# BBCG/epialleleR

Hardware: AMD Instinct MI355X
Metric: Mreads/s generateCytosineReport (150 bp PE) (higher is better)
Workload: dtype u8

## Files before the change

epialleler_amd/csrc/cx_report.hip:

```cpp
#include "common.hpp"
#include "tile_common.hpp"
#include <stdio.h>
#include <stdlib.h>
#include <string.h>

namespace epi {

#ifndef EPI_CX_WG
#define EPI_CX_WG 512
#endif
#ifndef EPI_CX_T1
#define EPI_CX_T1 2048
#endif
constexpr int CX_WG = EPI_CX_WG;
constexpr int CX_T1 = EPI_CX_T1;
constexpr int CX_CH = 16;
constexpr int CX_FLUSH_ROWS = 255;
constexpr int CX_SLAB_COV = 12;

struct __attribute__((packed, aligned(1))) U4u { uint32_t x, y, z, w; };

#ifndef EPI_CX_ABLATE
#define EPI_CX_ABLATE 0
#endif

struct Cx2Args {
  RowCols c;
  int64_t xm_cap;
  const Tile *tiles;
  uint32_t fill4;
  ClassLut lut_r;
  ClassLut lut_rx, lut_sx;
  ClassLut lut_s;
  ThrParams thr;
  const uint32_t *thr_tab;
  uint32_t ctx_of_plane;
  int32_t *pass_out;
  uint32_t *pool_key, *pool_meth, *pool_unmeth;
  uint32_t pool_cap;
  uint32_t *cursor;
  uint32_t slot_rows, ovf_base;
  uint32_t *tile_nrow, *tile_base;
  int32_t *slab;
  int heavy_rows;
  int heavy_chunk;
  int heavy_first;
  uint32_t *heavy_count, *heavy_max;
  uint32_t *heavy_list;
  int32_t *heavy_slab;
  uint32_t *deep_count, *deep_list;
  const uint32_t *tile_list, *tile_list_count;
  uint32_t *dbg;
  int64_t nrows;
  const uint32_t *prev_off, *prev_nrow;
  uint32_t *mismatch;
  int32_t *out[6];
  int64_t out_cap;
};

template <int T, int NP, bool LEAN = false> struct Cx2Lds {
  static constexpr int Q = T / 4;
  static constexpr int N_NARROW = 2 * NP * Q;
  static constexpr int N_CORR = 2 * Q;
  static constexpr int N_WIDE = LEAN ? 16 : 2 * NP * T;
  static constexpr int N_COV = T;
  unsigned long long *narrow, *corr;
  uint32_t *wide, *cov;
  uint32_t tid;
};

__device__ __forceinline__ uint32_t cx2_lut(uint32_t w, const ClassLut &X, uint32_t low8) {
  const uint32_t sel = (w & 0x0F0F0F0Fu) | low8;
  return __builtin_amdgcn_perm(X.lo1, X.lo0, sel) ^ __builtin_amdgcn_perm(X.hi1, X.hi0, sel ^ 0x08080808u);
}

template <int G>
__device__ __forceinline__ uint32_t cx2_group_sum(uint32_t v) {
  v += (uint32_t)__builtin_amdgcn_update_dpp(0, (int)v, 0xB1, 0xF, 0xF, true);
  v += (uint32_t)__builtin_amdgcn_update_dpp(0, (int)v, 0x4E, 0xF, 0xF, true);
  if (G >= 8) v += (uint32_t)__builtin_amdgcn_update_dpp(0, (int)v, 0x141, 0xF, 0xF, true);
  if (G >= 16) v += (uint32_t)__builtin_amdgcn_update_dpp(0, (int)v, 0x140, 0xF, 0xF, true);
  if (G >= 32) v += __shfl_xor(v, 16, 64);
  if (G >= 64) v += __shfl_xor(v, 32, 64);
  return v;
}

__device__ __forceinline__ int cx2_threshold(uint32_t n_m, uint32_t n_u, uint32_t o_m, uint32_t o_u, const ThrParams &prm) {
  int res = 0;
  if (n_m != 0) {
    const unsigned n_all = n_m + n_u;
    if (!(n_all < prm.min_n_ctx)) {
      const double frac = (double)n_m / (double)n_all;
      if (!(frac < prm.min_ctx_meth_frac)) {
        res = 1;
        if (o_m > 0) {
          const unsigned o_all = o_m + o_u;
          const double ofrac = (double)o_m / (double)o_all;
          if (ofrac > prm.max_ooctx_meth_frac) res = 0;
        }
      }
    }
  }
  return res;
}

__device__ __forceinline__ int cx2_threshold_tab(uint32_t n_m, uint32_t n_u, uint32_t o_m, uint32_t o_u, const ThrParams &prm,
                                                 const uint32_t *__restrict__ tab) {
  const uint32_t n_all = n_m + n_u, o_all = o_m + o_u;
  const uint32_t least = tab[n_all] & 0xFFFFu, most = tab[o_all] >> 16;
  return n_m != 0u && !(n_all < prm.min_n_ctx) && n_m >= least && (o_m == 0u || o_m <= most);
}

__global__ __launch_bounds__(256) void k_thr_table(ThrParams prm, int32_t nmax, uint32_t *__restrict__ tab) {
  const int32_t n = (int32_t)(blockIdx.x * 256 + threadIdx.x);
  if (n > nmax) return;
  uint32_t least = 0xFFFFu, most = 0u;
  if (n >= 1) {
    int32_t lo = 1, hi = n + 1;
    while (lo < hi) {
      const int32_t m = (lo + hi) >> 1;
      const double frac = (double)(uint32_t)m / (double)(uint32_t)n;
      if (!(frac < prm.min_ctx_meth_frac)) hi = m; else lo = m + 1;
    }
    if (lo <= n) least = (uint32_t)lo;
    lo = 1; hi = n + 1;
    while (lo < hi) {
      const int32_t m = (lo + hi) >> 1;
      const double frac = (double)(uint32_t)m / (double)(uint32_t)n;
      if (frac > prm.max_ooctx_meth_frac) hi = m; else lo = m + 1;
    }
    most = (uint32_t)(lo - 1);
  }
  tab[n] = least | (most << 16);
}

struct Cx2Row {
  const uint8_t *base;
  int32_t rel, len;
  int32_t c0, clast;
  bool edge;
  int sidx, ps;
};

__device__ __forceinline__ void cx2_mask_from(int lo , uint32_t (&m)[4]) {
  const unsigned long long x = ~0ull << ((8 * lo) & 63);
  const bool low = lo < 8;
  const unsigned long long a = low ? x : 0ull, b = low ? ~0ull : x;
  m[0] = (uint32_t)a; m[1] = (uint32_t)(a >> 32); m[2] = (uint32_t)b; m[3] = (uint32_t)(b >> 32);
// ... 59 lines not shown
    if (x == 0x12345678u) atomicAdd(L.cov, 1u);
    return;
  }
  {
    uint32_t mf[4], ml[4];
    cx2_mask_from(cb == g.c0 ? (g.rel & 15) : 0, mf);
    cx2_mask_upto(((g.rel + g.len - 1) & 15) + 1, ml);
#pragma unroll
    for (int d = 0; d < 4; d++) { asm("" : "+v"(mf[d])); asm("" : "+v"(ml[d])); }
#pragma unroll
    for (int d = 0; d < 4; d++) w[0][d] = (w[0][d] & mf[d]) | (a.fill4 & ~mf[d]);
#pragma unroll
    for (int u = 0; u < NU; u++) {
      const bool last = cb + u * G == g.clast;
      if (__ballot(last) != 0ull) {
        const uint32_t keep = last ? 0u : 0xFFFFFFFFu;
#pragma unroll
        for (int d = 0; d < 4; d++) {
          const uint32_t m = ml[d] | keep;
          w[u][d] = (w[u][d] & m) | (a.fill4 & ~m);
        }
      }
    }
  }

  unsigned long long *nar = L.narrow + g.sidx * NP * Q + 4 * cb;
  unsigned long long *cor = L.corr + g.sidx * Q + 4 * cb;
  if constexpr (FUSED) {
    static_assert(NP == 1, "fused thresholding: one reported context, the thresholding context");
    uint32_t cls[4] = {0, 0, 0, 0}, fl = 0;
#pragma unroll
    for (int u = 0; u < NU; u++) {
#pragma unroll
      for (int d = 0; d < 4; d++) w[u][d] = (EPI_CX_ABLATE & 4) ? w[u][d] : cx2_lut(w[u][d], a.lut_sx, 0u);
      fl |= w[u][0] | w[u][1] | w[u][2] | w[u][3];
    }
    auto count = [&](auto masked) {
      constexpr bool MASKED = decltype(masked)::value;
      constexpr uint32_t EV = MASKED ? 0x55555555u : 0xFFFFFFFFu;
      uint32_t E = 0, O = 0;
#pragma unroll
      for (int u = 0; u < NU; u++) {
        const uint32_t t = (w[u][0] & EV) + (w[u][1] & EV) + (w[u][2] & EV);
        const uint32_t d3 = w[u][3] & EV;
        E += (t & 0x33333333u) + (d3 & 0x33333333u);
        O += ((t >> 2) & 0x33333333u) + ((d3 >> 2) & 0x33333333u);
        if (u % 3 == 2 || u == NU - 1) {
          cls[0] = __builtin_amdgcn_sad_u8(E & 0x0F0F0F0Fu, 0u, cls[0]);
          cls[2] = __builtin_amdgcn_sad_u8((E >> 4) & 0x0F0F0F0Fu, 0u, cls[2]);
          cls[1] = __builtin_amdgcn_sad_u8(O & 0x0F0F0F0Fu, 0u, cls[1]);
          cls[3] = __builtin_amdgcn_sad_u8((O >> 4) & 0x0F0F0F0Fu, 0u, cls[3]);
          E = 0; O = 0;
        }
      }
    };
    if constexpr (MODE != 2) {
      if (__builtin_expect(__ballot((fl & 0xAAAAAAAAu) != 0u) == 0ull, 1)) count(std::false_type{});
      else count(std::true_type{});
    }
    if constexpr (MODE == 1) {
#pragma unroll
      for (int k = 0; k < 4; k++) carry[k] += cls[k];
      return;
    }
    if constexpr (MODE == 0) {
      const uint32_t s01 = cx2_group_sum<G>(cls[0] | (cls[1] << 16)), s23 = cx2_group_sum<G>(cls[2] | (cls[3] << 16));
      const uint32_t n_all = s01 & 0xFFFFu, n_m = s01 >> 16;
      g.ps = a.thr_tab ? cx2_threshold_tab(n_m, n_all - n_m, s23 & 0xFFFFu, s23 >> 16, a.thr, a.thr_tab)
                       : cx2_threshold(n_m, n_all - n_m, s23 & 0xFFFFu, s23 >> 16, a.thr);
      if (a.pass_out && sub == 0 && (uint32_t)g.rel < (uint32_t)T) a.pass_out[rcur] = g.ps;
    }
    const uint32_t pm = g.ps ? 0x01010101u : 0u;
#pragma unroll
    for (int u = 0; u < NU; u++) {
      const bool inside = (uint32_t)(cb + u * G) < (uint32_t)C;
#pragma unroll
      for (int d = 0; d < 4; d++) {
        const uint32_t lo = w[u][d] & 0x01010101u, hi = (w[u][d] >> 2) & pm;
        if (lo != 0u && inside && !(EPI_CX_ABLATE & 2)) atomicAdd(nar + 4 * u * G + d, (unsigned long long)lo | ((unsigned long long)hi << 32));
      }
    }
    const uint32_t fsel = g.ps ? 0x0A0A0A0Au : 0xA0A0A0A0u;
    if (__builtin_expect((fl & fsel) != 0u, 0)) {
      const int sh = g.ps ? 1 : 5;
#pragma unroll
      for (int u = 0; u < NU; u++) {
        const bool inside = (uint32_t)(cb + u * G) < (uint32_t)C;
#pragma unroll
        for (int d = 0; d < 4; d++) {
          const uint32_t sk = (w[u][d] >> sh) & 0x01010101u, db = (w[u][d] >> (sh + 2)) & 0x01010101u;
          if ((sk | db) != 0u && inside) atomicAdd(cor + 4 * u * G + d, (unsigned long long)sk | ((unsigned long long)db << 32));
        }
      }
    }
  } else if constexpr (NP == 1 && G >= 16) {
    const bool passing = g.ps != 0;
    const uint32_t k77 = (a.ctx_of_plane & 255u) * 0x11111111u;
    const uint32_t rm = passing ? 0xDDDDDDDDu : 0x55555555u, rv = passing ? 0x99999999u : 0x11111111u;
    uint32_t clean = 0xFFFFFFFFu;
#pragma unroll
    for (int u = 0; u < NU; u++) {
      const bool inside = (uint32_t)(cb + u * G) < (uint32_t)C;
#pragma unroll
      for (int e = 0; e < 2; e++) {
        const uint32_t pk = (w[u][2 * e] & 0x0F0F0F0Fu) | ((w[u][2 * e + 1] << 4) & 0xF0F0F0F0u);
        const uint32_t z = ((pk & 0x77777777u) ^ k77) + 0x77777777u;
        const uint32_t np = ~z & 0x88888888u;
        const uint32_t t = (pk & rm) ^ rv;
        clean &= ((t & 0x77777777u) + 0x77777777u) | t;
        if (np != 0u && inside && !(EPI_CX_ABLATE & 2)) {
          const uint32_t up = passing ? np & ~pk : 0u;
          const uint32_t n0 = (np >> 3) & 0x01010101u, n1 = (np >> 7) & 0x01010101u;
          if (n0 != 0u) atomicAdd(nar + 4 * u * G + 2 * e, (unsigned long long)n0 | ((unsigned long long)((up >> 3) & 0x01010101u) << 32));
          if (n1 != 0u) atomicAdd(nar + 4 * u * G + 2 * e + 1, (unsigned long long)n1 | ((unsigned long long)((up >> 7) & 0x01010101u) << 32));
        }
      }
    }
    if (__builtin_expect((~clean & 0x88888888u) != 0u, 0)) {
      const uint32_t pick0 = passing ? 0u : 0x08080808u;
#pragma unroll
      for (int u = 0; u < NU; u++) {
        const bool inside = (uint32_t)(cb + u * G) < (uint32_t)C;
#pragma unroll
        for (int d = 0; d < 4; d++) {
          const uint32_t f = cx2_lut(w[u][d], a.lut_rx, pick0);
          const uint32_t sk = (f >> 6) & 0x01010101u, db = (f >> 7) & 0x01010101u;
          if ((sk | db) != 0u && inside) atomicAdd(cor + 4 * u * G + d, (unsigned long long)sk | ((unsigned long long)db << 32));
        }
      }
    }
  } else {
    const uint32_t pick0 = g.ps == 0 ? 0x08080808u : 0u;
    uint32_t fl = 0;
#pragma unroll
    for (int u = 0; u < NU; u++) {
      const bool inside = (uint32_t)(cb + u * G) < (uint32_t)C;
#pragma unroll
      for (int d = 0; d < 4; d++) {
        const uint32_t f = cx2_lut(w[u][d], a.lut_rx, pick0);
        w[u][d] = f;
        fl |= f;
#pragma unroll
        for (int p = 0; p < NP; p++) {
          const uint32_t lo = (f >> (2 * p)) & 0x01010101u, hi = (f >> (2 * p + 1)) & 0x01010101u;
          if (lo != 0u && inside && !(EPI_CX_ABLATE & 2))
            atomicAdd(nar + p * Q + 4 * u * G + d, (unsigned long long)lo | ((unsigned long long)hi << 32));
        }
      }
    }
    if (__builtin_expect((fl & 0xC0C0C0C0u) != 0u, 0)) {
#pragma unroll
      for (int u = 0; u < NU; u++) {
        const bool inside = (uint32_t)(cb + u * G) < (uint32_t)C;
#pragma unroll
        for (int d = 0; d < 4; d++) {
          const uint32_t sk = (w[u][d] >> 6) & 0x01010101u, db = (w[u][d] >> 7) & 0x01010101u;
          if ((sk | db) != 0u && inside) atomicAdd(cor + 4 * u * G + d, (unsigned long long)sk | ((unsigned long long)db << 32));
        }
      }
    }
  }
}

template <int T, int G, int NU, int NP, bool FUSED, int WG, class LT>
__device__ __forceinline__ void cx2_rows(const Cx2Args &a, const Tile &td, int row_lo, int row_hi, const LT &L) {
  constexpr int R = 64 / G, NW = WG / 64, C = T / CX_CH;
  const int lane = L.tid & 63, wave = L.tid >> 6;
  const int sub = lane & (G - 1), grp = lane / G;
  Tile tb = td;
  tb.row_hi = row_hi;
  int r = row_lo + wave * R + grp;
  RowVals v = cx_load_row(a.c, tb, r);
  for (int rbase = row_lo + wave * R; rbase < row_hi; rbase += NW * R) {
    const int rcur = r;
    if (!EPI_DEV_CHECK(a.dbg, !v.ok || (rcur >= 0 && rcur < a.nrows && v.len >= 0 && (v.sd == 1 || v.sd == 2 || v.len == 0)), 22, rcur, v.sd)) return;
    r += NW * R;
    RowVals nv;
    bool fetched = false;
    auto fetch_next = [&]() { if (!fetched) { nv = cx_load_row(a.c, tb, r); fetched = true; } };
    if (v.ok && v.len > 0 && (int32_t)((uint32_t)v.st - (uint32_t)td.pos0) + v.len > 0) {
      Cx2Row g;
      g.rel = (int32_t)((uint32_t)v.st - (uint32_t)td.pos0);
      g.len = v.len;
      g.c0 = g.rel >> 4;
      g.clast = (g.rel + v.len - 1) >> 4;
      g.base = a.c.xm + (v.o - g.rel);
      g.edge = v.o < CX_CH || v.o + v.len + CX_CH > a.xm_cap;
      g.sidx = v.sd - 1;
      g.ps = v.ps;
      if constexpr (FUSED) {
        if (__builtin_expect(__ballot(g.clast - g.c0 >= G * NU) == 0ull, 1)) {
          cx2_visit<T, G, NU, NP, true>(a, g, g.c0, g.clast, sub, rcur, L, fetch_next);
        } else {
          uint32_t cls[4] = {0, 0, 0, 0};
          for (int32_t cs = g.c0; __ballot(cs <= g.clast) != 0ull; cs += G * NU)
            cx2_visit<T, G, NU, NP, true, 1>(a, g, cs, g.clast, sub, rcur, L, fetch_next, cls);
          const uint32_t s01 = cx2_group_sum<G>(cls[0] | (cls[1] << 16)), s23 = cx2_group_sum<G>(cls[2] | (cls[3] << 16));
          const uint32_t n_all = s01 & 0xFFFFu, n_m = s01 >> 16;
          g.ps = a.thr_tab ? cx2_threshold_tab(n_m, n_all - n_m, s23 & 0xFFFFu, s23 >> 16, a.thr, a.thr_tab)
                           : cx2_threshold(n_m, n_all - n_m, s23 & 0xFFFFu, s23 >> 16, a.thr);
          if (a.pass_out && sub == 0 && (uint32_t)g.rel < (uint32_t)T) a.pass_out[rcur] = g.ps;
          const int32_t ca = g.c0 > 0 ? g.c0 : 0, cz = g.clast < C - 1 ? g.clast : C - 1;
          for (int32_t cs = ca; __ballot(cs <= cz) != 0ull; cs += G * NU)
            cx2_visit<T, G, NU, NP, true, 2>(a, g, cs, cz, sub, rcur, L, fetch_next);
        }
      } else {
        const int32_t ca = g.c0 > 0 ? g.c0 : 0, cz = g.clast < C - 1 ? g.clast : C - 1;
        if (__builtin_expect(__ballot(cz - ca >= G * NU) == 0ull, 1)) {
          cx2_visit<T, G, NU, NP, false>(a, g, ca, cz, sub, rcur, L, fetch_next);
        } else {
          for (int32_t cs = ca; __ballot(cs <= cz) != 0ull; cs += G * NU) cx2_visit<T, G, NU, NP, false>(a, g, cs, cz, sub, rcur, L, fetch_next);
        }
      }
      if (sub == 0) {
        const int32_t ca = g.rel > 0 ? g.rel : 0, cb = g.rel + v.len < T ? g.rel + v.len : T;
        const uint32_t unit = g.sidx ? 65536u : 1u;
        if (ca < cb && !(EPI_CX_ABLATE & 32)) { atomicAdd(L.cov + ca, unit); if (cb < T) atomicAdd(L.cov + cb, 0u - unit); }
      }
    } else if (FUSED && v.ok && sub == 0 && a.pass_out && (uint32_t)((uint32_t)v.st - (uint32_t)td.pos0) < (uint32_t)T) {
      a.pass_out[rcur] = 0;
    }
    fetch_next();
    v = nv;
  }
}

template <int T, int NP, bool LEAN, int WG>
__device__ __forceinline__ void cx2_flush(const Cx2Lds<T, NP, LEAN> &L) {
  constexpr int Q = Cx2Lds<T, NP, LEAN>::Q;
  if constexpr (!LEAN) {
    for (int i = L.tid; i < 2 * NP * Q; i += WG) {
      const unsigned long long v = L.narrow[i];
      if (v == 0ull) continue;
      L.narrow[i] = 0ull;
      const uint32_t lo = (uint32_t)v, hi = (uint32_t)(v >> 32);
      const int sp = i / Q, q = i - sp * Q;
      uint4 *wd = reinterpret_cast<uint4 *>(L.wide + sp * T + 4 * q);
      uint4 c = *wd;
      c.x += (lo & 255u) | ((hi & 255u) << 16);
      c.y += ((lo >> 8) & 255u) | (((hi >> 8) & 255u) << 16);
      c.z += ((lo >> 16) & 255u) | (((hi >> 16) & 255u) << 16);
      c.w += (lo >> 24) | ((hi >> 24) << 16);
      *wd = c;
    }
  }
  for (int i = L.tid; i < 2 * Q; i += WG) {
    const unsigned long long v = L.corr[i];
    if (v == 0ull) continue;
    L.corr[i] = 0ull;
    const uint32_t sk = (uint32_t)v, db = (uint32_t)(v >> 32);
    const int s = i / Q, q = i - s * Q;
    const int32_t unit = s ? 65536 : 1;
    int32_t prev = 0;
#pragma unroll
    for (int j = 0; j < 4; j++) {
      const int32_t d = (int32_t)((db >> (8 * j)) & 255u) - (int32_t)((sk >> (8 * j)) & 255u);
      if (d != prev) atomicAdd(L.cov + 4 * q + j, (uint32_t)((d - prev) * unit));
      prev = d;
    }
    if (prev != 0 && 4 * q + 4 < T) atomicAdd(L.cov + 4 * q + 4, (uint32_t)(-prev * unit));
  }
}

__device__ __forceinline__ uint32_t cx_pool_reserve(const Cx2Args &a, int tile, uint32_t n, bool *fits) {
  if (n <= a.slot_rows) { *fits = true; return (uint32_t)tile * a.slot_rows; }
  const uint32_t o = atomicAdd(a.cursor, n);
  *fits = (uint64_t)a.ovf_base + o + n <= a.pool_cap;
  return a.ovf_base + o;
}

__device__ __forceinline__ void cx_direct_none(const Cx2Args &a, int tile, uint32_t tid = threadIdx.x) {
  if (a.prev_off && tid == 0 && a.prev_nrow[tile] != 0u) atomicAdd(a.mismatch, 1u);
}

template <int T, int NP> struct CxSrcLds {
  const uint32_t *wide, *cov;
  __device__ __forceinline__ uint32_t any(int sd, int pos) const {
    uint32_t x = 0;
#pragma unroll
    for (int p = 0; p < NP; p++) x |= wide[(sd * NP + p) * T + pos];
    return x;
  }
  __device__ __forceinline__ void pair(int sd, int p, int pos, uint32_t *n, uint32_t *M) const {
    const uint32_t w = wide[(sd * NP + p) * T + pos];
    *n = w & 0xFFFFu; *M = w >> 16;
  }
  __device__ __forceinline__ uint32_t coverage(int sd, int pos) const { const uint32_t v = cov[pos]; return sd ? v >> 16 : v & 0xFFFFu; }
};
template <int QS> struct CxSrcU8 {
  const uint32_t *narrow;
  const uint32_t *cov;
  __device__ __forceinline__ uint32_t any(int sd, int pos) const {
    return (narrow[2 * (sd * QS + (pos >> 2))] >> (8 * (pos & 3))) & 255u;
  }
  __device__ __forceinline__ void pair(int sd, int, int pos, uint32_t *n, uint32_t *M) const {
    const uint2 c = *reinterpret_cast<const uint2 *>(narrow + 2 * (sd * QS + (pos >> 2)));
    *n = (c.x >> (8 * (pos & 3))) & 255u; *M = (c.y >> (8 * (pos & 3))) & 255u;
  }
  __device__ __forceinline__ uint32_t coverage(int sd, int pos) const { const uint32_t v = cov[pos]; return sd ? v >> 16 : v & 0xFFFFu; }
};
template <int T, int NP> struct CxSrcSlab {
  const int32_t *slab;
  const uint32_t *cov;
  __device__ __forceinline__ uint32_t any(int sd, int pos) const {
    uint32_t x = 0;
#pragma unroll
    for (int p = 0; p < NP; p++) x |= (uint32_t)slab[(2 * (sd * NP + p)) * T + pos];
    return x;
  }
  __device__ __forceinline__ void pair(int sd, int p, int pos, uint32_t *n, uint32_t *M) const {
    *n = (uint32_t)slab[(2 * (sd * NP + p)) * T + pos]; *M = (uint32_t)slab[(2 * (sd * NP + p) + 1) * T + pos];
  }
  __device__ __forceinline__ uint32_t coverage(int sd, int pos) const { return cov[sd * T + pos]; }
};

template <int T, int WG = CX_WG>
__device__ __forceinline__ void cx2_prefix(uint32_t *arr, uint32_t *s_scan, uint32_t tid = threadIdx.x) {
  constexpr int PPT = T / WG, NW = WG / 64;
  static_assert(PPT >= 1 && PPT <= 8, "prefix layout");
  const int lane = tid & 63, wave = tid >> 6;
  uint32_t x[PPT];
#pragma unroll
  for (int j = 0; j < PPT; j++) x[j] = arr[tid * PPT + j];
#pragma unroll
  for (int j = 1; j < PPT; j++) x[j] += x[j - 1];
  const uint32_t inc = wave_scan_u32(x[PPT - 1]);
  if (lane == 63) s_scan[wave] = inc;
  __syncthreads();
  uint32_t before = inc - x[PPT - 1];
#pragma unroll
  for (int w = 0; w < NW; w++) before += w < wave ? s_scan[w] : 0u;
#pragma unroll
  for (int j = 0; j < PPT; j++) arr[tid * PPT + j] = x[j] + before;
  __syncthreads();
}

template <int T, int NP, int WG = CX_WG, class SRC>
__device__ __forceinline__ void cx2_emit(const Cx2Args &a, int tile, const SRC &src, uint32_t *s_scan, uint16_t *s_list, uint32_t tid = threadIdx.x) {
  constexpr int NW = WG / 64, PW = T / NW, IT = PW / 32;
  static_assert(PW % 32 == 0 && IT >= 1 && IT <= 16, "emit phase layout");
  const int lane = tid & 63, wave = tid >> 6;
  const int l5 = lane & 31, sd = lane >> 5;
  const uint32_t below = (1u << l5) - 1u;
  uint16_t *list = s_list + wave * (2 * PW);
  uint32_t nc = 0;
#pragma unroll
  for (int i = 0; i < IT; i++) {
    const uint32_t any = src.any(sd, wave * PW + i * 32 + l5);
    const unsigned long long bal = __ballot(any != 0u);
    const uint32_t blo = (uint32_t)bal, bhi = (uint32_t)(bal >> 32);
    const uint32_t rank = (uint32_t)__popc(blo & below) + (uint32_t)__popc(bhi & below) + (sd ? (blo >> l5) & 1u : 0u);
    if (any != 0u) list[nc + rank] = (uint16_t)(i * 64 + lane);
    nc += (uint32_t)__popcll(bal);
  }
  uint32_t key[IT], me[IT], un[IT], off[IT];
  bool ok[IT];
  uint32_t carry = 0;
#pragma unroll
  for (int jj = 0; jj < IT; jj++) {
    ok[jj] = false; key[jj] = 0; me[jj] = 0; un[jj] = 0; off[jj] = 0;
    if ((uint32_t)(jj * 64) < nc) {
      const uint32_t j = (uint32_t)(jj * 64 + lane);
      bool good = false;
      if (j < nc) {
        const uint32_t id = list[j];
        const int pos = wave * PW + (int)(id >> 6) * 32 + (int)(id & 31u), st = (int)((id >> 5) & 1u);
        const uint32_t half = src.coverage(st, pos) >> 1;
        uint32_t ctx = 0, m = 0, u = 0;
#pragma unroll
        for (int p = 0; p < NP; p++) {
          uint32_t nn, M;
          src.pair(st, p, pos, &nn, &M);
          if (nn > half && ctx == 0) { ctx = (a.ctx_of_plane >> (8 * p)) & 255u; m = M; u = nn - M; }
        }
        good = ctx != 0;
        key[jj] = ((uint32_t)pos << 4) | ((uint32_t)st << 3) | ctx;
        me[jj] = m;
        un[jj] = u;
      }
      const unsigned long long be = __ballot(good);
      off[jj] = carry + __builtin_amdgcn_mbcnt_hi((uint32_t)(be >> 32), __builtin_amdgcn_mbcnt_lo((uint32_t)be, 0u));
      carry += (uint32_t)__popcll(be);
      ok[jj] = good;
    }
  }
  if (lane == 0) s_scan[wave] = carry;
  __syncthreads();
  if (a.prev_off) {
    if (tid == 0) {
      uint32_t acc = 0;
      for (int w = 0; w < NW; w++) { const uint32_t t = s_scan[w]; s_scan[w] = acc; acc += t; }
      const uint32_t base = a.prev_off[tile];
      const bool good = acc == a.prev_nrow[tile] && (int64_t)base + acc <= a.out_cap;
      if (!good) atomicAdd(a.mismatch, 1u);
      s_scan[NW + 1] = good ? base : 0xFFFFFFFFu;
    }
    __syncthreads();
    const uint32_t base = s_scan[NW + 1];
    if (base != 0xFFFFFFFFu) {
      const Tile td = a.tiles[tile];
      const uint32_t w0 = base + s_scan[wave];
#pragma unroll
      for (int jj = 0; jj < IT; jj++) {
        if (ok[jj]) {
          const uint32_t o = w0 + off[jj];
          a.out[0][o] = td.rname;
          a.out[1][o] = 1 + (int32_t)((key[jj] >> 3) & 1u);
          a.out[2][o] = (int32_t)(td.pos0 + (int64_t)(key[jj] >> 4));
          a.out[3][o] = (int32_t)(key[jj] & 7u);
          a.out[4][o] = (int32_t)me[jj];
          a.out[5][o] = (int32_t)un[jj];
        }
      }
    }
    return;
  }
  if (tid == 0) {
    uint32_t acc = 0;
    for (int w = 0; w < NW; w++) { const uint32_t t = s_scan[w]; s_scan[w] = acc; acc += t; }
    s_scan[NW] = acc;
    uint32_t base = 0;
    bool fits = true;
    if (acc) base = cx_pool_reserve(a, tile, acc, &fits);
    s_scan[NW + 1] = base;
    s_scan[NW] = fits ? acc : 0xFFFFFFFFu;
    a.tile_nrow[tile] = acc;
    a.tile_base[tile] = base;
  }
  __syncthreads();
  const uint32_t total = s_scan[NW], base = s_scan[NW + 1];
  if (total != 0xFFFFFFFFu) {
    const uint32_t w0 = base + s_scan[wave];
#pragma unroll
    for (int jj = 0; jj < IT; jj++) {
      if (ok[jj]) {
        const uint32_t w = w0 + off[jj];
        if (!EPI_DEV_CHECK(a.dbg, w < a.pool_cap, 23, w, a.pool_cap)) continue;
        a.pool_key[w] = key[jj];
        a.pool_meth[w] = me[jj];
        a.pool_unmeth[w] = un[jj];
      }
    }
  }
}

template <int T, int NP, bool LEAN, int WG>
__device__ __forceinline__ void cx2_dump_slab(const Cx2Lds<T, NP, LEAN> &L, int32_t *slab) {
  uint32_t *dst = reinterpret_cast<uint32_t *>(slab);
  if constexpr (LEAN) {
    constexpr int Q = Cx2Lds<T, NP, LEAN>::Q;
    for (int i = L.tid; i < 2 * NP * Q; i += WG) {
      const unsigned long long v = L.narrow[i];
      if (v == 0ull) continue;
      const uint32_t lo = (uint32_t)v, hi = (uint32_t)(v >> 32);
      const int sp = i / Q, q = i - sp * Q;
#pragma unroll
      for (int j = 0; j < 4; j++) {
        const uint32_t n = (lo >> (8 * j)) & 255u, M = (hi >> (8 * j)) & 255u;
        if (n) atomicAdd(dst + (2 * sp) * T + 4 * q + j, n);
        if (M) atomicAdd(dst + (2 * sp + 1) * T + 4 * q + j, M);
      }
    }
  } else {
    for (int i = L.tid; i < 2 * NP * T; i += WG) {
      const uint32_t v = L.wide[i];
      if (!v) continue;
      const int sp = i / T, p = i - sp * T;
      if (v & 0xFFFFu) atomicAdd(dst + (2 * sp) * T + p, v & 0xFFFFu);
      if (v >> 16) atomicAdd(dst + (2 * sp + 1) * T + p, v >> 16);
    }
  }
  for (int p = L.tid; p < T; p += WG) {
    const uint32_t v = L.cov[p];
    if (!v) continue;
    const int32_t lo = (int32_t)(int16_t)(v & 0xFFFFu);
    const int32_t hi = ((int32_t)v - lo) >> 16;
    if (lo) atomicAdd(dst + CX_SLAB_COV * T + p, (uint32_t)lo);
    if (hi) atomicAdd(dst + (CX_SLAB_COV + 1) * T + p, (uint32_t)hi);
  }
}

__device__ __forceinline__ int cx_tile_of_block(int b, int ntiles) {
  const int chunk = (ntiles + 7) >> 3;
  return (b & 7) * chunk + (b >> 3);
}

template <int T, int NP, bool LEAN = false> constexpr int cx2_lds_bytes() {
  using LdsT = Cx2Lds<T, NP, LEAN>;
  return (LdsT::N_NARROW + LdsT::N_CORR) * 8 + (LdsT::N_WIDE + LdsT::N_COV) * 4;
}
#ifndef EPI_CX_WPS
#define EPI_CX_WPS 8
#endif
template <int T, int NP, int NU = 3, bool LEAN = false, int WG = CX_WG> constexpr int cx2_waves_per_simd() {
  const int by_lds = (160 * 1024) / (cx2_lds_bytes<T, NP, LEAN>() + 64), by_thr = 2048 / WG;
  int wgs = by_lds < by_thr ? by_lds : by_thr;
  if (NU >= 4 && wgs * WG > 1536) wgs = 1536 / WG;
  if (wgs * WG / 256 > EPI_CX_WPS) wgs = EPI_CX_WPS * 256 / WG;
  return (wgs < 1 ? 1 : wgs) * WG / 256;
}

#define CX2_SHARED(T, NP, LEAN)                                                                                  \
  using LdsT = Cx2Lds<T, NP, LEAN>;                                                                              \
  __shared__ __attribute__((aligned(16))) unsigned long long s_u8[LdsT::N_NARROW + LdsT::N_CORR];                \
  __shared__ __attribute__((aligned(16))) uint32_t s_wide[LdsT::N_WIDE];                                         \
  __shared__ __attribute__((aligned(16))) uint32_t s_cov[LdsT::N_COV];                                           \
  static_assert((LdsT::N_NARROW + LdsT::N_CORR) * 8 >= 4 * T + 64 && LdsT::N_CORR * 8 >= 4 * T, "the candidate lists and the scan scratch reuse dead arrays"); \
  uint32_t *s_scan = LEAN ? s_wide : reinterpret_cast<uint32_t *>(s_u8) + T;                                      \
  uint16_t *s_list = reinterpret_cast<uint16_t *>(LEAN ? s_u8 + LdsT::N_NARROW : s_u8);                          \
  (void)s_scan; (void)s_list;                                                                                     \
  LdsT L;                                                                                                         \
  L.narrow = s_u8; L.corr = s_u8 + LdsT::N_NARROW; L.wide = s_wide; L.cov = s_cov; L.tid = threadIdx.x;

template <int T, int NP, bool LEAN, int WG>
__device__ __forceinline__ void cx2_clear(const Cx2Lds<T, NP, LEAN> &L) {
  using LdsT = Cx2Lds<T, NP, LEAN>;
  uint4 *z = reinterpret_cast<uint4 *>(L.narrow);
  for (int i = L.tid; i < (LdsT::N_NARROW + LdsT::N_CORR) / 2; i += WG) z[i] = make_uint4(0, 0, 0, 0);
  if constexpr (!LEAN) {
    uint4 *y = reinterpret_cast<uint4 *>(L.wide);
    for (int i = L.tid; i < LdsT::N_WIDE / 4; i += WG) y[i] = make_uint4(0, 0, 0, 0);
  }
  uint4 *x = reinterpret_cast<uint4 *>(L.cov);
  for (int i = L.tid; i < LdsT::N_COV / 4; i += WG) x[i] = make_uint4(0, 0, 0, 0);
}

template <int T, int G, int NU, int NP, bool FUSED, bool LEAN, int WG>
__device__ __forceinline__ void cx2_accumulate(const Cx2Args &a, const Tile &td, int row_lo, int row_hi, const Cx2Lds<T, NP, LEAN> &L) {
  if constexpr (LEAN) {
    cx2_rows<T, G, NU, NP, FUSED, WG>(a, td, row_lo, row_hi, L);
  } else {
    for (int b0 = row_lo; b0 < row_hi; b0 += CX_FLUSH_ROWS) {
      if (b0 > row_lo) { __syncthreads(); cx2_flush<T, NP, LEAN, WG>(L); __syncthreads(); }
      cx2_rows<T, G, NU, NP, FUSED, WG>(a, td, b0, b0 + CX_FLUSH_ROWS < row_hi ? b0 + CX_FLUSH_ROWS : row_hi, L);
    }
  }
  __syncthreads();
  cx2_flush<T, NP, LEAN, WG>(L);
  __syncthreads();
}

#ifndef EPI_CX_LEAN_WG
#define EPI_CX_LEAN_WG 256
#endif
template <bool LEAN> constexpr int cx2_wg() { return LEAN ? EPI_CX_LEAN_WG : CX_WG; }

template <int T, int G, int NU, int NP, bool FUSED, bool LEAN, class LdsT>
__device__ __forceinline__ void cx2_tile(const Cx2Args &a, int tile, const Tile &td, const LdsT &L, uint32_t *s_scan, uint16_t *s_list, int *s_flag) {
  constexpr int WG = cx2_wg<LEAN>();
  cx2_clear<T, NP, LEAN, WG>(L);
  if (td.row_hi - td.row_lo > a.heavy_rows) {
    if (L.tid == 0) {
      const uint32_t h = atomicAdd(a.heavy_count, 1u);
      a.heavy_list[h] = (uint32_t)tile;
      atomicMax(a.heavy_max, (uint32_t)(td.row_hi - td.row_lo));
      a.tile_nrow[tile] = 0;
      a.tile_base[tile] = 0;
    }
    cx_direct_none(a, tile, L.tid);
    return;
  }
  if constexpr (LEAN) {
    if (a.deep_list && td.row_hi - td.row_lo > CX_FLUSH_ROWS) {
      if (L.tid == 0) *s_flag = 0;
      __syncthreads();
      bool deep = false;
      for (int x = td.row_lo + (int)L.tid; x + CX_FLUSH_ROWS < td.row_hi; x += WG)
        deep |= (int64_t)a.c.start[x + CX_FLUSH_ROWS] < (int64_t)a.c.start[x] + a.c.len[x];
      if (deep) *s_flag = 1;
      __syncthreads();
      if (*s_flag) {
        if (L.tid == 0) { a.deep_list[atomicAdd(a.deep_count, 1u)] = (uint32_t)tile; a.tile_nrow[tile] = 0; a.tile_base[tile] = 0; }
        cx_direct_none(a, tile, L.tid);
        return;
      }
    }
  }
  __syncthreads();
  cx2_accumulate<T, G, NU, NP, FUSED, LEAN, WG>(a, td, td.row_lo, td.row_hi, L);
  if (td.slot >= 0) {
    cx2_dump_slab<T, NP, LEAN, WG>(L, a.slab + (int64_t)td.slot * (kCxPlanes * T));
    if (L.tid == 0) { a.tile_nrow[tile] = 0; a.tile_base[tile] = 0; }
    cx_direct_none(a, tile, L.tid);
    return;
  }
  if (EPI_CX_ABLATE & 16) { if (L.tid == 0) { a.tile_nrow[tile] = 0; a.tile_base[tile] = 0; } cx_direct_none(a, tile, L.tid); return; }
  cx2_prefix<T, WG>(L.cov, s_scan, L.tid);
  if constexpr (LEAN) {
    static_assert(NP == 1, "the u8 counters serve single-context reports");
    CxSrcU8<LdsT::Q> src;
    src.narrow = reinterpret_cast<const uint32_t *>(L.narrow); src.cov = L.cov;
    cx2_emit<T, NP, WG>(a, tile, src, s_scan, s_list, L.tid);
  } else {
    CxSrcLds<T, NP> src;
    src.wide = L.wide; src.cov = L.cov;
    cx2_emit<T, NP, WG>(a, tile, src, s_scan, s_list, L.tid);
  }
}

template <int T, int G, int NU, int NP, bool FUSED, bool LEAN>
__global__ __launch_bounds__(cx2_wg<LEAN>(), (cx2_waves_per_simd<T, NP, NU, LEAN, cx2_wg<LEAN>()>())) void k_cx_tiles(Cx2Args a, int ntiles) {
  CX2_SHARED(T, NP, LEAN)
  __shared__ int s_flag;
  if constexpr (!LEAN) {
    if (a.tile_list) {
      const uint32_t n = *a.tile_list_count;
      for (uint32_t i = blockIdx.x; i < n; i += gridDim.x) {
        const int tile = (int)a.tile_list[i];
        const Tile td = a.tiles[tile];
        cx2_tile<T, G, NU, NP, FUSED, LEAN>(a, tile, td, L, s_scan, s_list, &s_flag);
        __syncthreads();
      }
      return;
    }
  }
  const int tile = cx_tile_of_block(blockIdx.x, ntiles);
  if (tile >= ntiles) return;
  const Tile td = a.tiles[tile];
  cx2_tile<T, G, NU, NP, FUSED, LEAN>(a, tile, td, L, s_scan, s_list, &s_flag);
}

template <int T, int G, int NU, int NP, bool FUSED>
__global__ __launch_bounds__(CX_WG, (cx2_waves_per_simd<T, NP, NU>())) void k_cx_heavy(Cx2Args a) {
  CX2_SHARED(T, NP, false)
  const uint32_t hi_idx = (uint32_t)a.heavy_first + blockIdx.y;
  if (hi_idx >= *a.heavy_count) return;
  const int tile = (int)a.heavy_list[hi_idx];
  const Tile td = a.tiles[tile];
  for (int lo = td.row_lo + (int)blockIdx.x * a.heavy_chunk; lo < td.row_hi; lo += (int)gridDim.x * a.heavy_chunk) {
    const int hi = td.row_hi - lo > a.heavy_chunk ? lo + a.heavy_chunk : td.row_hi;
    cx2_clear<T, NP, false, CX_WG>(L);
    __syncthreads();
    cx2_accumulate<T, G, NU, NP, FUSED, false, CX_WG>(a, td, lo, hi, L);
    cx2_dump_slab<T, NP, false, CX_WG>(L, td.slot >= 0 ? a.slab + (int64_t)td.slot * (kCxPlanes * T)
                                          : a.heavy_slab + (int64_t)blockIdx.y * (kCxPlanes * T));
    __syncthreads();
  }
}

template <int T, int NP>
__device__ __forceinline__ void cx2_emit_from_slab(const Cx2Args &a, int tile, const int32_t *slab) {
  __shared__ __attribute__((aligned(16))) uint32_t s_cov[2 * T];
  __shared__ uint32_t s_scan[CX_WG / 64 + 2];
  __shared__ uint16_t s_list[2 * T];
  for (int i = threadIdx.x; i < 2 * T; i += CX_WG) s_cov[i] = (uint32_t)slab[CX_SLAB_COV * T + i];
  __syncthreads();
  cx2_prefix<T>(s_cov, s_scan);
  cx2_prefix<T>(s_cov + T, s_scan);
  CxSrcSlab<T, NP> src;
  src.slab = slab; src.cov = s_cov;
  cx2_emit<T, NP>(a, tile, src, s_scan, s_list);
}

template <int T, int NP>
__global__ __launch_bounds__(CX_WG) void k_cx_emit_heavy(Cx2Args a) {
  const uint32_t hi_idx = (uint32_t)a.heavy_first + blockIdx.x;
  if (hi_idx >= *a.heavy_count) return;
  const int tile = (int)a.heavy_list[hi_idx];
  if (a.tiles[tile].slot >= 0) return;
  cx2_emit_from_slab<T, NP>(a, tile, a.heavy_slab + (int64_t)blockIdx.x * (kCxPlanes * T));
}

template <int T, int NP>
__global__ __launch_bounds__(CX_WG) void k_cx_emit_slab(Cx2Args a, const int32_t *__restrict__ owned,
                                                         const int32_t *__restrict__ slot_tile) {
  if (!owned[blockIdx.x]) return;
  const int tile = slot_tile[blockIdx.x];
  if (tile < 0) return;
  cx2_emit_from_slab<T, NP>(a, tile, a.slab + (int64_t)a.tiles[tile].slot * (kCxPlanes * T));
}

#ifndef EPI_CXP_T
#define EPI_CXP_T 1024
#endif
constexpr int CXP_T = EPI_CXP_T;

template <int G, int U0, int U1>
__device__ __forceinline__ void cxp_add_range(const uint32_t (&w)[CX_NU], const RowSlice &cur) {
  if constexpr (U0 < U1) {
    if (U0 * G <= cur.tl) cx_add_dword<CXP_T, 4 * G * U0, U0 == 0>(w[U0], cur.tl == U0 * G, cur);
    cxp_add_range<G, U0 + 1, U1>(w, cur);
  }
}

template <int G>
__device__ __forceinline__ void cxp_accumulate(const RowCols &c, const Tile &td, uint32_t *cnt) {
  constexpr int R = 64 / G, NW = CX_WG / 64;
  const int lane = threadIdx.x & 63, wave = threadIdx.x >> 6;
  const int sub = lane & (G - 1), grp = lane / G;
  int r = td.row_lo + wave * R + grp;
  RowSlice cur = cx_row_slice<CXP_T, G>(c, td, r, sub, cnt);
  for (int rbase = td.row_lo + wave * R; rbase < td.row_hi; rbase += NW * R) {
    uint32_t w[CX_NU];
#pragma unroll
    for (int u = 0; u < CX_NU; u++) w[u] = u * G <= cur.tl ? cur.src[u * G] : 0u;
    r += NW * R;
    const RowSlice nxt = cx_row_slice<CXP_T, G>(c, td, r, sub, cnt);
    cxp_add_range<G, 0, CX_NU>(w, cur);
    for (int k = sub + CX_NU * G; k < cur.nd; k += G) {
      RowSlice t = cur;
#pragma unroll
      for (int j = 0; j < 4; j++) t.dst[j] = cur.dst[j] + 4 * (k - sub);
      cx_add_dword<CXP_T, 0, false>(cur.src[k - sub], k == cur.nd - 1, t);
    }
    cur = nxt;
  }
}

__device__ __forceinline__ void cxp_convert(uint32_t *cnt) {
  constexpr int T = CXP_T;
  for (int i = threadIdx.x; i < 2 * T; i += CX_WG) {
    uint32_t *c0 = cnt + (i / T) * 4 * T + (i % T);
    const uint32_t d0 = c0[0], dh = c0[T], dx = c0[2 * T], dz = c0[3 * T];
    const uint32_t nh = (dh & 0xFFFFu) + (dh >> 16), nx = (dx & 0xFFFFu) + (dx >> 16), nz = (dz & 0xFFFFu) + (dz >> 16);
    c0[0] = (d0 & 0xFFFFu) + (d0 >> 16) + nh + nx + nz;
    c0[T] = nh | (dh << 16);
    c0[2 * T] = nx | (dx << 16);
    c0[3 * T] = nz | (dz << 16);
  }
}

struct CxSrcPk {
  const uint32_t *cnt;
  int pl[3];
  __device__ __forceinline__ uint32_t any(int sd, int pos) const {
    uint32_t x = 0;
#pragma unroll
    for (int p = 0; p < 3; p++) if (pl[p]) x |= cnt[(sd * 4 + pl[p]) * CXP_T + pos];
    return x;
  }
  __device__ __forceinline__ void pair(int sd, int p, int pos, uint32_t *n, uint32_t *M) const {
    const uint32_t w = pl[p] ? cnt[(sd * 4 + pl[p]) * CXP_T + pos] : 0u;
    *n = w & 0xFFFFu; *M = w >> 16;
  }
  __device__ __forceinline__ uint32_t coverage(int sd, int pos) const { return cnt[sd * 4 * CXP_T + pos]; }
};

__device__ __forceinline__ CxSrcPk cxp_source(const Cx2Args &a, const uint32_t *cnt) {
  CxSrcPk s;
  s.cnt = cnt;
#pragma unroll
  for (int p = 0; p < 3; p++) { const uint32_t k = (a.ctx_of_plane >> (8 * p)) & 255u; s.pl[p] = k == 2u ? 1 : k == 6u ? 2 : k == 7u ? 3 : 0; }
  return s;
}

__device__ __forceinline__ void cxp_dump_slab(const Cx2Args &a, const uint32_t *cnt, int np, int32_t *slab) {
  constexpr int T = CXP_T;
  uint32_t *dst = reinterpret_cast<uint32_t *>(slab);
  const CxSrcPk src = cxp_source(a, cnt);
  for (int i = threadIdx.x; i < 2 * T; i += CX_WG) {
    const int sd = i / T, pos = i % T;
#pragma unroll
    for (int p = 0; p < 3; p++) {
      if (p >= np) break;
      uint32_t n, M;
      src.pair(sd, p, pos, &n, &M);
      if (n) atomicAdd(dst + (2 * (sd * np + p)) * T + pos, n);
      if (M) atomicAdd(dst + (2 * (sd * np + p) + 1) * T + pos, M);
    }
    const uint32_t d = src.coverage(sd, pos) - (pos ? src.coverage(sd, pos - 1) : 0u);
    if (d) atomicAdd(dst + (CX_SLAB_COV + sd) * T + pos, d);
  }
}

#define CXP_SHARED                                                                                      \
  __shared__ __attribute__((aligned(16))) uint32_t cnt_raw[8 * CXP_T + 2 * kCxGuard];                  \
  __shared__ uint32_t s_scan[CX_WG / 64 + 2];                                                         \
  __shared__ uint16_t s_list[2 * CXP_T];                                                               \
  uint32_t *cnt = cnt_raw + kCxGuard;

template <int G>
__global__ __launch_bounds__(CX_WG, 8) void k_cxp_tiles(Cx2Args a, int ntiles, int np) {
  CXP_SHARED
  const int tile = cx_tile_of_block(blockIdx.x, ntiles);
  if (tile >= ntiles) return;
  const Tile td = a.tiles[tile];
  uint4 *z = reinterpret_cast<uint4 *>(cnt_raw);
  for (int i = threadIdx.x; i < (8 * CXP_T + 2 * kCxGuard) / 4; i += CX_WG) z[i] = make_uint4(0, 0, 0, 0);
  if (td.row_hi - td.row_lo > a.heavy_rows) {
    if (threadIdx.x == 0) {
      const uint32_t h = atomicAdd(a.heavy_count, 1u);
      a.heavy_list[h] = (uint32_t)tile;
      atomicMax(a.heavy_max, (uint32_t)(td.row_hi - td.row_lo));
      a.tile_nrow[tile] = 0;
      a.tile_base[tile] = 0;
    }
    cx_direct_none(a, tile);
    return;
  }
  __syncthreads();
  cxp_accumulate<G>(a.c, td, cnt);
  __syncthreads();
  cxp_convert(cnt);
  __syncthreads();
  if (td.slot >= 0) {
    cxp_dump_slab(a, cnt, np, a.slab + (int64_t)td.slot * (kCxPlanes * CXP_T));
    if (threadIdx.x == 0) { a.tile_nrow[tile] = 0; a.tile_base[tile] = 0; }
    cx_direct_none(a, tile);
    return;
  }
  if (EPI_CX_ABLATE & 16) {
    if (threadIdx.x == 0) { a.tile_nrow[tile] = 0; a.tile_base[tile] = 0; }
    cx_direct_none(a, tile);
    return;
  }
  cx2_emit<CXP_T, 3>(a, tile, cxp_source(a, cnt), s_scan, s_list);
}

template <int G>
__global__ __launch_bounds__(CX_WG, 8) void k_cxp_heavy(Cx2Args a, int np) {
  CXP_SHARED
  (void)s_scan; (void)s_list;
  const uint32_t hi_idx = (uint32_t)a.heavy_first + blockIdx.y;
  if (hi_idx >= *a.heavy_count) return;
  const int tile = (int)a.heavy_list[hi_idx];
  const Tile whole = a.tiles[tile];
  for (int lo = whole.row_lo + (int)blockIdx.x * a.heavy_chunk; lo < whole.row_hi; lo += (int)gridDim.x * a.heavy_chunk) {
    Tile td = whole;
    td.row_lo = lo;
    if (td.row_hi - lo > a.heavy_chunk) td.row_hi = lo + a.heavy_chunk;
    uint4 *z = reinterpret_cast<uint4 *>(cnt_raw);
    for (int i = threadIdx.x; i < (8 * CXP_T + 2 * kCxGuard) / 4; i += CX_WG) z[i] = make_uint4(0, 0, 0, 0);
    __syncthreads();
    cxp_accumulate<G>(a.c, td, cnt);
    __syncthreads();
    cxp_convert(cnt);
    __syncthreads();
    cxp_dump_slab(a, cnt, np, td.slot >= 0 ? a.slab + (int64_t)td.slot * (kCxPlanes * CXP_T)
                                            : a.heavy_slab + (int64_t)blockIdx.y * (kCxPlanes * CXP_T));
    __syncthreads();
  }
}

struct __attribute__((packed, aligned(4))) CxU4u { uint32_t x, y, z, w; };

__global__ __launch_bounds__(256) void k_cx_gather(const Tile *__restrict__ tiles, const uint32_t *__restrict__ tile_out,
                                                    const uint32_t *__restrict__ tile_nrow, const uint32_t *__restrict__ tile_base,
                                                    int32_t ntiles, const uint32_t *__restrict__ pool_key,
                                                    const uint32_t *__restrict__ pool_meth, const uint32_t *__restrict__ pool_unmeth,
                                                    int32_t *__restrict__ o_rname, int32_t *__restrict__ o_strand,
                                                    int32_t *__restrict__ o_pos, int32_t *__restrict__ o_ctx,
                                                    int32_t *__restrict__ o_meth, int32_t *__restrict__ o_unmeth) {
  const int tile = blockIdx.x * 4 + (threadIdx.x >> 6);
  if (tile >= ntiles) return;
  const uint32_t n = tile_nrow[tile];
  if (n == 0) return;
  const int lane = threadIdx.x & 63;
  const Tile td = tiles[tile];
  const uint32_t src0 = tile_base[tile], dst0 = tile_out[tile];
  const uint32_t n4 = n & ~3u;
  for (uint32_t i = 4u * lane; i < n4; i += 256) {
    const CxU4u key = *reinterpret_cast<const CxU4u *>(pool_key + src0 + i);
    const CxU4u me = *reinterpret_cast<const CxU4u *>(pool_meth + src0 + i);
    const CxU4u un = *reinterpret_cast<const CxU4u *>(pool_unmeth + src0 + i);
    const uint32_t o = dst0 + i;
    const uint32_t rn = (uint32_t)td.rname;
    const uint32_t p0 = (uint32_t)td.pos0;
    *reinterpret_cast<CxU4u *>(o_rname + o) = CxU4u{rn, rn, rn, rn};
    *reinterpret_cast<CxU4u *>(o_strand + o) = CxU4u{1u + ((key.x >> 3) & 1u), 1u + ((key.y >> 3) & 1u), 1u + ((key.z >> 3) & 1u), 1u + ((key.w >> 3) & 1u)};
    *reinterpret_cast<CxU4u *>(o_pos + o) = CxU4u{p0 + (key.x >> 4), p0 + (key.y >> 4), p0 + (key.z >> 4), p0 + (key.w >> 4)};
    *reinterpret_cast<CxU4u *>(o_ctx + o) = CxU4u{key.x & 7u, key.y & 7u, key.z & 7u, key.w & 7u};
    *reinterpret_cast<CxU4u *>(o_meth + o) = me;
    *reinterpret_cast<CxU4u *>(o_unmeth + o) = un;
  }
  for (uint32_t i = n4 + lane; i < n; i += 64) {
    const uint32_t key = pool_key[src0 + i];
    const uint32_t o = dst0 + i;
    o_rname[o] = td.rname;
    o_strand[o] = 1 + (int32_t)((key >> 3) & 1u);
    o_pos[o] = (int32_t)(td.pos0 + (int64_t)(key >> 4));
    o_ctx[o] = (int32_t)(key & 7u);
    o_meth[o] = (int32_t)pool_meth[src0 + i];
    o_unmeth[o] = (int32_t)pool_unmeth[src0 + i];
  }
}


static int cx_tile_for(int np) { return np <= 1 ? CX_T1 : CXP_T; }

static int pick_cx_shape(const RowStats &st, int T, bool fused, bool lean) {
#ifdef EPI_CX_FORCE_SHAPE
  if (fused) return EPI_CX_FORCE_SHAPE;
#endif
  const int max_chunks = (int)(((int64_t)st.max_len + 2 * (CX_CH - 1)) / CX_CH);
  const int tile_chunks = T / CX_CH;
  double total = 0;
  for (int k = 0; k < kLenBinCount; k++) total += st.len_hist[k];
  int best = 64 * 8 + 3;
  double best_cost = -1;
// ... 662 lines not shown
```

Measured before the change: 12820.

## Skip lean correction flush when unused; hoist kept-offset loads and drop emit barrier

Adds an LDS flag in the lean layout that records whether any correction atomics fired, and skips the flush pass and its barrier when none did. The per-tile previous offset and row count are now loaded once at kernel entry and passed into emit. The serial thread-0 scan in emit, with its extra __syncthreads, is replaced by each wave reading all wave totals itself. The goal is fewer barriers and less serialized global traffic per tile, at the cost of some redundant LDS reads and added flag-store complexity.

Result: slower. 12120 (-5.5%).

```diff
diff --git a/epialleler_amd/csrc/cx_report.hip b/epialleler_amd/csrc/cx_report.hip
--- a/epialleler_amd/csrc/cx_report.hip
+++ b/epialleler_amd/csrc/cx_report.hip
@@ -64,6 +64,8 @@
   static constexpr int N_CORR = 2 * Q;
   static constexpr int N_WIDE = LEAN ? 16 : 2 * NP * T;
   static constexpr int N_COV = T;
+  static constexpr bool kLean = LEAN;
+  static constexpr int CORR_FLAG = 15;
   unsigned long long *narrow, *corr;
   uint32_t *wide, *cov;
   uint32_t tid;
@@ -289,6 +291,7 @@
     }
     const uint32_t fsel = g.ps ? 0x0A0A0A0Au : 0xA0A0A0A0u;
     if (__builtin_expect((fl & fsel) != 0u, 0)) {
+      if constexpr (LT::kLean) L.wide[LT::CORR_FLAG] = 1u;
       const int sh = g.ps ? 1 : 5;
 #pragma unroll
       for (int u = 0; u < NU; u++) {
@@ -324,6 +327,7 @@
       }
     }
     if (__builtin_expect((~clean & 0x88888888u) != 0u, 0)) {
+      if constexpr (LT::kLean) L.wide[LT::CORR_FLAG] = 1u;
       const uint32_t pick0 = passing ? 0u : 0x08080808u;
 #pragma unroll
       for (int u = 0; u < NU; u++) {
@@ -356,6 +360,7 @@
       }
     }
     if (__builtin_expect((fl & 0xC0C0C0C0u) != 0u, 0)) {
+      if constexpr (LT::kLean) L.wide[LT::CORR_FLAG] = 1u;
 #pragma unroll
       for (int u = 0; u < NU; u++) {
         const bool inside = (uint32_t)(cb + u * G) < (uint32_t)C;
@@ -480,6 +485,13 @@
   if (a.prev_off && tid == 0 && a.prev_nrow[tile] != 0u) atomicAdd(a.mismatch, 1u);
 }
 
+struct CxKept { uint32_t off, nrow; };
+__device__ __forceinline__ CxKept cx_kept(const Cx2Args &a, int tile) {
+  CxKept k = {0u, 0u};
+  if (a.prev_off) { k.off = a.prev_off[tile]; k.nrow = a.prev_nrow[tile]; }
+  return k;
+}
+
 template <int T, int NP> struct CxSrcLds {
   const uint32_t *wide, *cov;
   __device__ __forceinline__ uint32_t any(int sd, int pos) const {
@@ -543,7 +555,8 @@
 }
 
 template <int T, int NP, int WG = CX_WG, class SRC>
-__device__ __forceinline__ void cx2_emit(const Cx2Args &a, int tile, const SRC &src, uint32_t *s_scan, uint16_t *s_list, uint32_t tid = threadIdx.x) {
+__device__ __forceinline__ void cx2_emit(const Cx2Args &a, int tile, const CxKept &kept, int32_t rname, int64_t pos0, const SRC &src,
+                                         uint32_t *s_scan, uint16_t *s_list, uint32_t tid = threadIdx.x) {
   constexpr int NW = WG / 64, PW = T / NW, IT = PW / 32;
   static_assert(PW % 32 == 0 && IT >= 1 && IT <= 16, "emit phase layout");
   const int lane = tid & 63, wave = tid >> 6;
@@ -594,30 +607,24 @@
   if (lane == 0) s_scan[wave] = carry;
   __syncthreads();
   if (a.prev_off) {
-    if (tid == 0) {
-      uint32_t acc = 0;
-      for (int w = 0; w < NW; w++) { const uint32_t t = s_scan[w]; s_scan[w] = acc; acc += t; }
-      const uint32_t base = a.prev_off[tile];
-      const bool good = acc == a.prev_nrow[tile] && (int64_t)base + acc <= a.out_cap;
-      if (!good) atomicAdd(a.mismatch, 1u);
-      s_scan[NW + 1] = good ? base : 0xFFFFFFFFu;
-    }
-    __syncthreads();
-    const uint32_t base = s_scan[NW + 1];
-    if (base != 0xFFFFFFFFu) {
-      const Tile td = a.tiles[tile];
-      const uint32_t w0 = base + s_scan[wave];
-#pragma unroll
-      for (int jj = 0; jj < IT; jj++) {
-        if (ok[jj]) {
-          const uint32_t o = w0 + off[jj];
-          a.out[0][o] = td.rname;
-          a.out[1][o] = 1 + (int32_t)((key[jj] >> 3) & 1u);
-          a.out[2][o] = (int32_t)(td.pos0 + (int64_t)(key[jj] >> 4));
-          a.out[3][o] = (int32_t)(key[jj] & 7u);
-          a.out[4][o] = (int32_t)me[jj];
-          a.out[5][o] = (int32_t)un[jj];
-        }
+    uint32_t before = 0, total = 0;
+#pragma unroll
+    for (int w = 0; w < NW; w++) { const uint32_t t = s_scan[w]; before += w < wave ? t : 0u; total += t; }
+    if (total != kept.nrow || (int64_t)kept.off + total > a.out_cap) {
+      if (tid == 0) atomicAdd(a.mismatch, 1u);
+      return;
+    }
+    const uint32_t w0 = kept.off + before;
+#pragma unroll
+    for (int jj = 0; jj < IT; jj++) {
+      if (ok[jj]) {
+        const uint32_t o = w0 + off[jj];
+        a.out[0][o] = rname;
+        a.out[1][o] = 1 + (int32_t)((key[jj] >> 3) & 1u);
+        a.out[2][o] = (int32_t)(pos0 + (int64_t)(key[jj] >> 4));
+        a.out[3][o] = (int32_t)(key[jj] & 7u);
+        a.out[4][o] = (int32_t)me[jj];
+        a.out[5][o] = (int32_t)un[jj];
       }
     }
     return;
@@ -730,6 +737,7 @@
   }
   uint4 *x = reinterpret_cast<uint4 *>(L.cov);
   for (int i = L.tid; i < LdsT::N_COV / 4; i += WG) x[i] = make_uint4(0, 0, 0, 0);
+  if constexpr (LEAN) { if (L.tid == 0) L.wide[LdsT::CORR_FLAG] = 0u; }
 }
 
 template <int T, int G, int NU, int NP, bool FUSED, bool LEAN, int WG>
@@ -743,6 +751,9 @@
     }
   }
   __syncthreads();
+  if constexpr (LEAN) {
+    if (td.slot < 0 && __builtin_amdgcn_readfirstlane(L.wide[Cx2Lds<T, NP, LEAN>::CORR_FLAG]) == 0u) return;
+  }
   cx2_flush<T, NP, LEAN, WG>(L);
   __syncthreads();
 }
@@ -753,8 +764,10 @@
 template <bool LEAN> constexpr int cx2_wg() { return LEAN ? EPI_CX_LEAN_WG : CX_WG; }
 
 template <int T, int G, int NU, int NP, bool FUSED, bool LEAN, class LdsT>
-__device__ __forceinline__ void cx2_tile(const Cx2Args &a, int tile, const Tile &td, const LdsT &L, uint32_t *s_scan, uint16_t *s_list, int *s_flag) {
+__device__ __forceinline__ void cx2_tile(const Cx2Args &a, int tile, const Tile &td, const CxKept &kept, const LdsT &L, uint32_t *s_scan,
+                                         uint16_t *s_list, int *s_flag) {
   constexpr int WG = cx2_wg<LEAN>();
+  static_assert(!LEAN || WG / 64 + 2 <= LdsT::CORR_FLAG, "the scan scratch and the corr flag share the `wide` stub");
   cx2_clear<T, NP, LEAN, WG>(L);
   if (td.row_hi - td.row_lo > a.heavy_rows) {
     if (L.tid == 0) {
@@ -797,11 +810,11 @@
     static_assert(NP == 1, "the u8 counters serve single-context reports");
     CxSrcU8<LdsT::Q> src;
     src.narrow = reinterpret_cast<const uint32_t *>(L.narrow); src.cov = L.cov;
-    cx2_emit<T, NP, WG>(a, tile, src, s_scan, s_list, L.tid);
+    cx2_emit<T, NP, WG>(a, tile, kept, td.rname, td.pos0, src, s_scan, s_list, L.tid);
   } else {
     CxSrcLds<T, NP> src;
     src.wide = L.wide; src.cov = L.cov;
-    cx2_emit<T, NP, WG>(a, tile, src, s_scan, s_list, L.tid);
+    cx2_emit<T, NP, WG>(a, tile, kept, td.rname, td.pos0, src, s_scan, s_list, L.tid);
   }
 }
 
@@ -815,7 +828,8 @@
       for (uint32_t i = blockIdx.x; i < n; i += gridDim.x) {
         const int tile = (int)a.tile_list[i];
         const Tile td = a.tiles[tile];
-        cx2_tile<T, G, NU, NP, FUSED, LEAN>(a, tile, td, L, s_scan, s_list, &s_flag);
+        const CxKept kept = cx_kept(a, tile);
+        cx2_tile<T, G, NU, NP, FUSED, LEAN>(a, tile, td, kept, L, s_scan, s_list, &s_flag);
         __syncthreads();
       }
       return;
@@ -824,7 +838,8 @@
   const int tile = cx_tile_of_block(blockIdx.x, ntiles);
   if (tile >= ntiles) return;
   const Tile td = a.tiles[tile];
-  cx2_tile<T, G, NU, NP, FUSED, LEAN>(a, tile, td, L, s_scan, s_list, &s_flag);
+  const CxKept kept = cx_kept(a, tile);
+  cx2_tile<T, G, NU, NP, FUSED, LEAN>(a, tile, td, kept, L, s_scan, s_list, &s_flag);
 }
 
 template <int T, int G, int NU, int NP, bool FUSED>
@@ -850,13 +865,15 @@
   __shared__ __attribute__((aligned(16))) uint32_t s_cov[2 * T];
   __shared__ uint32_t s_scan[CX_WG / 64 + 2];
   __shared__ uint16_t s_list[2 * T];
+  const Tile td = a.tiles[tile];
+  const CxKept kept = cx_kept(a, tile);
   for (int i = threadIdx.x; i < 2 * T; i += CX_WG) s_cov[i] = (uint32_t)slab[CX_SLAB_COV * T + i];
   __syncthreads();
   cx2_prefix<T>(s_cov, s_scan);
   cx2_prefix<T>(s_cov + T, s_scan);
   CxSrcSlab<T, NP> src;
   src.slab = slab; src.cov = s_cov;
-  cx2_emit<T, NP>(a, tile, src, s_scan, s_list);
+  cx2_emit<T, NP>(a, tile, kept, td.rname, td.pos0, src, s_scan, s_list);
 }
 
 template <int T, int NP>
@@ -982,6 +999,7 @@
   const int tile = cx_tile_of_block(blockIdx.x, ntiles);
   if (tile >= ntiles) return;
   const Tile td = a.tiles[tile];
+  const CxKept kept = cx_kept(a, tile);
   uint4 *z = reinterpret_cast<uint4 *>(cnt_raw);
   for (int i = threadIdx.x; i < (8 * CXP_T + 2 * kCxGuard) / 4; i += CX_WG) z[i] = make_uint4(0, 0, 0, 0);
   if (td.row_hi - td.row_lo > a.heavy_rows) {
@@ -1011,7 +1029,7 @@
     cx_direct_none(a, tile);
     return;
   }
-  cx2_emit<CXP_T, 3>(a, tile, cxp_source(a, cnt), s_scan, s_list);
+  cx2_emit<CXP_T, 3>(a, tile, kept, td.rname, td.pos0, cxp_source(a, cnt), s_scan, s_list);
 }
 
 template <int G>
```
